# SimonRennotte/Data-Efficient-Reinforcement-Learning-with-Probabilistic-Model-Predictive-Control

Hardware: AMD Instinct MI355X
Metric: MPC trajectory rollouts/sec (higher is better)
Workload: dtype f64

## Files before the change

### data-efficient-reinforcement-learning-with-probabilistic-model-predictive-control_amd/csrc/rollout_kernel.h

```cpp
#pragma once
#include "device_common.h"

#if defined(GPMPC_PROF_ON)
#define GPMPC_TRACE(id) do { if (threadIdx.x == 0 && blockIdx.x == 0) { long long now_ = __builtin_readcyclecounter(); \
    prof_acc[id] += now_ - prof_last; prof_last = now_; } \
    if (CL && threadIdx.x == 0 && (blockIdx.x & 7) == 0) { long long w_ = wall_clock64(); prof_wall[id] += w_ - prof_wlast; prof_wlast = w_; } } while (0)
#else
#define GPMPC_TRACE(id) do {} while (0)
#endif

namespace gpmpc_hip {

typedef const __attribute__((address_space(3))) double* lds_cptr;
__device__ inline double lds_b64(const double* p) {
    lds_cptr q = (lds_cptr)p;
    asm volatile("" : "+v"(q));
    return *q;
}

typedef double lds_d2 __attribute__((ext_vector_type(2)));
template <int NL, int NV>
__device__ inline void lds_load_pairs(const double* rec, double (&v)[NV]) {
    static_assert(NV >= ((NL + 1) & ~1), "destination too short");
    const lds_d2* r2 = reinterpret_cast<const lds_d2*>(rec);
#pragma unroll
    for (int k = 0; k < (NL + 1) / 2; ++k) { const lds_d2 t = r2[k]; v[2 * k] = t.x; v[2 * k + 1] = t.y; }
}

template <int DP>
struct RowRecPacked {
    static constexpr int RS = DP + 2, EA = 0, RA = 1, G = 2;
    template <int NL>
    static __device__ inline void load(const double* rec, double (&v)[RS]) {
#pragma unroll
        for (int k = 0; k < NL; ++k) v[k] = rec[k];
    }
};
template <int DP>
struct RowRecAligned {
    static constexpr int RS = (DP + 3) & ~1, EA = DP, RA = DP + 1, G = 0;
    template <int NL>
    static __device__ inline void load(const double* rec, double (&v)[RS]) { lds_load_pairs<NL>(rec, v); }
};

constexpr int kMaxTaylor = 14;
constexpr int kMaxMono = 256;

constexpr int kLaneMapSlots = 32;
constexpr int kLaneMapSlotsCluster = 192;
__host__ __device__ inline int tri_ints(int N) { return (N + 7) / 8 + 2; }

struct Layout {
    int mu, Sig, m, M, cc, s1, Vs, Sp, misc, rdet, aug, part, mom, ints, lmap, cl;
    int c_ils2, c_logvar, c_var, c_xr, c_act, c_exptab, c_monow, c_monoe, c_X;
    int lds_total;
    int nu, lb, rows, kb;
    int pp_total;
};

__host__ __device__ inline int rnd2(int x) { return (x + 1) & ~1; }

constexpr int kClusterScratch = 16 * 64 / 8;

__host__ __device__ inline Layout make_layout(int N, int D, int A, int E, int G, int DP, int wpp, int CM, int CH, int HA,
                                              bool x_in_lds, bool cluster = false, int lds_pairs = 0) {
    const int GL = (cluster && lds_pairs > 0) ? lds_pairs : G;
    Layout L;
    const int P = D * (D + 1) / 2;
    int o = 0;
    L.mu = o;   o += rnd2(D);
    L.Sig = o;  o += 2 * rnd2(D * D);
    L.m = o;    o += rnd2(E);
    L.M = o;    o += rnd2(D);
    L.cc = o;   o += rnd2(D);
    L.s1 = o;   o += rnd2(D * (D + 1));
    L.Vs = o;   o += rnd2(D * D);
    L.Sp = o;   o += rnd2(P);
    L.misc = o; o += 8;
    L.rdet = o; o += rnd2(G);
    L.aug = o;  o += (D + G) * 2 * D * D;
    L.part = o; o += rnd2(G * wpp);
    L.mom = o;  o += G * 2 * rnd2(CM);
    L.ints = o; o += rnd2((2 * P + 3 * G + 8 + 16 + tri_ints(N) + 1) / 2) + rnd2((D + G * wpp + 3) / 4);
    const int lms = cluster ? kLaneMapSlotsCluster : kLaneMapSlots;
    L.lmap = o; o += rnd2(((wpp < lms ? wpp : lms) * 65 + 1) / 2);
    L.cl = o;       o += cluster ? rnd2(G) + rnd2((G + 1) / 2) + 2 + kClusterScratch + rnd2((G * wpp + 2 * G + 16 + 7) / 8) +
                                   rnd2((G * wpp + 16 + 4 + 3) / 4) + rnd2((G + 1) / 2) + rnd2(G) : 0;
    L.c_ils2 = o;   o += rnd2(D * E);
    L.c_logvar = o; o += rnd2(D);
    L.c_var = o;    o += rnd2(D);
    L.c_xr = o;     o += rnd2(2 * E);
    L.c_act = o;    o += rnd2(HA);
    L.c_exptab = o; o += 64;
    L.c_monow = o;  o += rnd2(CM);
    L.c_monoe = o;  o += rnd2((CM + 1) / 2);
    L.c_X = o;      o += x_in_lds ? rnd2(E * N) : 0;
    int q = o;
    L.nu = q;   q += rnd2(D * N);
    L.lb = q;   q += rnd2(D * N);
    L.rows = q; q += GL * (N + CH) * ((DP + 3) & ~1);
    L.kb = q;   q += rnd2(GL * N);
    L.lds_total = q;
    L.pp_total = q - o;
    return L;
}

__device__ inline double gauss_solve(double* aug, int D, int nrhs, int ld) {
    double det = 1.0;
    const int nc = D + nrhs;
    for (int k = 0; k < D; ++k) {
        int piv = k;
        double best = fabs(aug[k * ld + k]);
        for (int r = k + 1; r < D; ++r) {
            double v = fabs(aug[r * ld + k]);
            if (v > best) { best = v; piv = r; }
        }
        if (piv != k) {
            for (int c = k; c < nc; ++c) {
                double t = aug[k * ld + c];
                aug[k * ld + c] = aug[piv * ld + c];
                aug[piv * ld + c] = t;
            }
            det = -det;
        }
        const double pv = aug[k * ld + k];
        det *= pv;
        const double ip = 1.0 / pv;
        for (int r = k + 1; r < D; ++r) {
            const double f = aug[r * ld + k] * ip;
            for (int c = k + 1; c < nc; ++c) aug[r * ld + c] -= f * aug[k * ld + c];
        }
    }
    for (int k = D - 1; k >= 0; --k) {
        const double ip = 1.0 / aug[k * ld + k];
        for (int c = D; c < nc; ++c) {
            double s = aug[k * ld + c];
            for (int r = k + 1; r < D; ++r) s -= aug[k * ld + r] * aug[r * ld + c];
            aug[k * ld + c] = s * ip;
        }
    }
    return det;
}

template <int DP>
__device__ inline double gauss_solve_reg(double (&a)[DP][2 * DP]) {
    double det = 1.0;
#pragma unroll
    for (int k = 0; k < DP; ++k) {
        int piv = k;
        double best = fabs(a[k][k]);
#pragma unroll
        for (int r = k + 1; r < DP; ++r) {
            const double v = fabs(a[r][k]);
            const bool better = v > best;
            best = better ? v : best;
            piv = better ? r : piv;
        }
#pragma unroll
        for (int r = k + 1; r < DP; ++r) {
            const bool sw = (piv == r);
#pragma unroll
            for (int c = 0; c < 2 * DP; ++c) {
                const double x = a[k][c], y = a[r][c];
                a[k][c] = sw ? y : x;
                a[r][c] = sw ? x : y;
            }
// ... 418 lines not shown
            const double(&grp)[16] = *reinterpret_cast<const double(*)[16]>(&acc[g16]);
            const double tot = wave_reduce16(grp);
            if ((lane & 3) == 0 && g16 + mq < NBm) mom[canon.v[g16 + mq]] = tot;
        }
        if constexpr (NP % 16 != 0) {
            constexpr int g8 = NP - 8;
            const double(&grp)[8] = *reinterpret_cast<const double(*)[8]>(&acc[g8]);
            const double tot = wave_reduce8(grp);
            if ((lane & 3) == 0 && lane < 32 && g8 + mq < NBm) mom[canon.v[g8 + mq]] = tot;
        }
    }
}

template <int KS>
__device__ __attribute__((noinline)) void sep3_item(int band, int lane, int N, int side, const double* rec0, int RS,
                                                     const double* kb, const double* nu, const double* il, double* mom) {
    switch (band) {
        case 0: sep3_band<KS, 0>(lane, N, side, rec0, RS, kb, nu, il, mom); break;
        case 1: sep3_band<KS, 1>(lane, N, side, rec0, RS, kb, nu, il, mom); break;
        case 2: sep3_band<KS, 2>(lane, N, side, rec0, RS, kb, nu, il, mom); break;
        case 3: sep3_band<KS, 3>(lane, N, side, rec0, RS, kb, nu, il, mom); break;
        case 4: sep3_band<KS, 4>(lane, N, side, rec0, RS, kb, nu, il, mom); break;
        case 5: sep3_band<KS, 5>(lane, N, side, rec0, RS, kb, nu, il, mom); break;
        default: sep3_band<KS, 6>(lane, N, side, rec0, RS, kb, nu, il, mom); break;
    }
}

template <int DP, bool CL>
constexpr int rollout_min_waves() { return (DP == 2 || (DP == 3 && !CL)) ? 4 : (DP == 6 ? 3 : 1); }

template <int DP, int NT, int DX, bool C2, bool TILED = false, bool CL = false>
__global__ __launch_bounds__(NT, (rollout_min_waves<DP, CL>())) void rollout_kernel(const RolloutArgs p) {
    static_assert(!TILED || (DP <= 4 && NT >= 256), "the batch-major path is built for D <= 4");
    static_assert(!CL || (!TILED && DP <= 4 && NT >= 256), "the cooperative form is built for D <= 4");
    extern __shared__ __attribute__((aligned(16))) double smem[];
    if constexpr (TILED) {
        if (p.slow[blockIdx.x] != p.t_begin + 1) return;
    }
    constexpr int NW = NT / kWave;
    using REC = RowRecAligned<DP>;
    constexpr int RS = REC::RS;
    const int tid = threadIdx.x;
    const int CS = CL ? p.cluster : 1;
    const bool spread = CL && (p.cl_dbg & 8);
    const int member = CL ? (spread ? (int)blockIdx.x % CS : (int)(blockIdx.x >> 3) % CS) : 0;
    const int c = CL ? (spread ? (int)blockIdx.x / CS : (int)(blockIdx.x & 7) + 8 * ((int)(blockIdx.x >> 3) / CS)) : (int)blockIdx.x;
    if constexpr (CL) { if (c >= p.B) return; }
    constexpr bool kMerged = !CL && DX > 0 && DP <= 4;
    constexpr bool kTailInTrip = DX == 0 || DP > 4;
    const int D = (DX > 0) ? DX : p.D;
    const int N = p.N, A = p.A, E = p.E, H = p.H, G = p.G, CM = p.CM;
    const int P = TILED ? D * (D - 1) / 2 : D * (D + 1) / 2;
    const int DA = D + A;
    const int LD = 2 * D;
    const int NC = C2 ? (N + 1) / 2 : N;
    const int wpp = (p.RC * NC + 63) / 64;
    const int SD2 = rnd2(D * D);

    const Layout L = make_layout(N, D, A, E, G, DP, wpp, CM, p.CH, H * A, p.x_in_lds != 0, CL, CL ? p.cl_slots : 0);
    const int NR = N + p.CH;
    double* s_mu = smem + L.mu;
    double* s_Sig2 = smem + L.Sig;
    double* s_m = smem + L.m;
    double* s_M = smem + L.M;
    double* s_cc = smem + L.cc;
    double* s_s1 = smem + L.s1;
    double* s_Vs = smem + L.Vs;
    double* s_Sp = smem + L.Sp;
    double* s_rdet = smem + L.rdet;
    [[maybe_unused]] double* s_rdiag = smem + L.misc;
    double* s_aug = smem + L.aug;
    double* s_part = smem + L.part;
    double* s_mom = smem + L.mom;
    int* s_pa = reinterpret_cast<int*>(smem + L.ints);
    int* s_pb = s_pa + P;
    int* s_K = s_pb + P;
    int* s_counter = s_K + G;
    int* s_noff = s_counter + 1;
    int* s_off = s_noff + 1;
    int* s_mcum = s_off + G;
    int* s_tri = s_mcum + 16;
    int* s_nslot = s_tri + tri_ints(N);
    int* s_nitems = s_nslot + G;
    unsigned short* s_items = reinterpret_cast<unsigned short*>(
        smem + L.ints + rnd2((2 * P + 3 * G + 8 + 16 + tri_ints(N) + 1) / 2));

    [[maybe_unused]] double* s_sepv = smem + L.cl;
    [[maybe_unused]] int* s_ord = reinterpret_cast<int*>(smem + L.cl + rnd2(G));
    [[maybe_unused]] int* s_fail = reinterpret_cast<int*>(smem + L.cl + rnd2(G) + rnd2((G + 1) / 2));
    [[maybe_unused]] unsigned char* s_needw = reinterpret_cast<unsigned char*>(smem + L.cl + rnd2(G) + rnd2((G + 1) / 2) + 2);
    [[maybe_unused]] unsigned char* s_own = s_needw + kClusterScratch * 8;
    [[maybe_unused]] unsigned char* s_sepown = s_own + G * wpp;
    [[maybe_unused]] unsigned char* s_elneed = s_sepown + G;
    [[maybe_unused]] unsigned char* s_meanown = s_elneed + G;
    [[maybe_unused]] unsigned short* s_mine = reinterpret_cast<unsigned short*>(
        smem + L.cl + rnd2(G) + rnd2((G + 1) / 2) + 2 + kClusterScratch + rnd2((G * wpp + 2 * G + 16 + 7) / 8));
    [[maybe_unused]] int* s_slot = reinterpret_cast<int*>(smem + L.cl + rnd2(G) + rnd2((G + 1) / 2) + 2 + kClusterScratch +
                                                          rnd2((G * wpp + 2 * G + 16 + 7) / 8) + rnd2((G * wpp + 16 + 4 + 3) / 4));
    [[maybe_unused]] unsigned long long* s_mymask = reinterpret_cast<unsigned long long*>(
        smem + L.cl + rnd2(G) + rnd2((G + 1) / 2) + 2 + kClusterScratch + rnd2((G * wpp + 2 * G + 16 + 7) / 8) +
        rnd2((G * wpp + 16 + 4 + 3) / 4) + rnd2((G + 1) / 2));
    const int GL = CL ? p.cl_slots : G;

    [[maybe_unused]] unsigned long long* xbuf_uc = CL ? p.xch_uc + (size_t)c * 4 * p.xch_n : nullptr;
    [[maybe_unused]] unsigned long long* xbuf = CL ? p.xch + (size_t)c * 4 * p.xch_n : nullptr;
    [[maybe_unused]] const int x_sep = G * wpp, x_mean = G * wpp + G;
    [[maybe_unused]] const int x_xcc = x_mean + D * (D + 1);
    [[maybe_unused]] int* s_lmap = reinterpret_cast<int*>(smem + L.lmap);
    constexpr int LMS = CL ? kLaneMapSlotsCluster : kLaneMapSlots;
    [[maybe_unused]] int* s_lrows = s_lmap + (wpp < LMS ? wpp : LMS) * 64;
    double* ppbase = smem;
    double* a_nu = ppbase + L.nu;
    double* a_lb = ppbase + L.lb;
    double* a_rows = ppbase + L.rows;
    double* a_kb = ppbase + L.kb;

    double* c_ils2 = smem + L.c_ils2;
    double* c_logvar = smem + L.c_logvar;
    double* c_var = smem + L.c_var;
    double* c_xr = smem + L.c_xr;
    double* c_act = smem + L.c_act;
    double* c_exptab = smem + L.c_exptab;
    const double* Xs = p.x_in_lds ? (smem + L.c_X) : p.Xt;
    double* c_monow = smem + L.c_monow;
    int* c_monoe = reinterpret_cast<int*>(smem + L.c_monoe);
    const double* act = p.actions + (size_t)c * H * A;

#if defined(GPMPC_PROF_ON)
    long long prof_left = 0;
    long long prof_acc[10] = {0, 0, 0, 0, 0, 0, 0, 0, 0, 0};
    long long prof_last = __builtin_readcyclecounter();
    long long prof_wall[10] = {0, 0, 0, 0, 0, 0, 0, 0, 0, 0};
    long long prof_wlast = wall_clock64();
    long long prof_b3 = 0, prof_chain = 0;
    int prof_chain_n = 0;
#endif
    if constexpr (TILED) {
        for (int i = tid; i < D; i += NT) { s_mu[i] = p.mu_out[((size_t)c * (H + 1) + p.t_begin) * D + i]; c_logvar[i] = p.logvar[i]; c_var[i] = p.var[i]; }
        for (int i = tid; i < D * D; i += NT) s_Sig2[i] = p.Sig_out[((size_t)c * (H + 1) + p.t_begin) * D * D + i];
    }
    {
        const bool inl = p.act_inline_n > 0;
        const int CMc = CM > 0 ? CM : 0;
        const double* mw = CMc > 0 ? p.mono_w : p.ils2;
        const int* me = CMc > 0 ? p.mono_exp : reinterpret_cast<const int*>(p.ils2);
        const int im = tid < CMc ? tid : 0;
        const int nX = p.x_in_lds ? E * N : 0;
        __builtin_amdgcn_sched_barrier(0);
        const double v_lv = p.logvar[tid < D ? tid : 0], v_var = p.var[tid < D ? tid : 0];
        const double v_ils = p.ils2[tid < D * E ? tid : 0], v_xr = p.xrange[tid < 2 * E ? tid : 0];
        const double v_act = act[tid < H * A ? tid : 0];
        const double v_exp = kExp2Tab[tid & 63];
        const double v_mw = mw[im];
        const int e0 = me[im * 4], e1 = me[im * 4 + 1], e2 = me[im * 4 + 2], e3 = me[im * 4 + 3];
        const double v_x0 = p.Xt[tid < nX ? tid : 0], v_x1 = p.Xt[tid + NT < nX ? tid + NT : 0];
        [[maybe_unused]] const double v_mu0 = p.mu0[tid < D ? tid : 0], v_S0 = p.S0[tid < D * D ? tid : 0];
        __builtin_amdgcn_sched_barrier(0);
        if constexpr (!TILED) {
            if (tid < D) s_mu[tid] = v_mu0;
            if (tid < D * D) s_Sig2[tid] = v_S0;
        }
        if (tid < D) { c_logvar[tid] = v_lv; c_var[tid] = v_var; }
        if (tid < D * E) c_ils2[tid] = v_ils;
        if (tid < 2 * E) c_xr[tid] = v_xr;
        if (tid < 64) c_exptab[tid] = v_exp;
        if (tid < CMc) { c_monow[tid] = v_mw; c_monoe[tid] = e0 | (e1 << 8) | (e2 << 16) | (e3 << 24); }
        if (tid < nX) smem[L.c_X + tid] = v_x0;
        if (tid + NT < nX) smem[L.c_X + tid + NT] = v_x1;
        if (inl) {
            for (int i = tid; i < H * A; i += NT) {
                const double v = p.act_inline[i < kInlineActs ? i : 0];
                c_act[i] = v;
                if (!CL || member == 0) p.act_store[i] = v;
            }
        } else {
            if (tid < H * A) c_act[tid] = v_act;
            for (int i = tid + NT; i < H * A; i += NT) c_act[i] = act[i];
        }
        for (int i = tid + NT; i < D; i += NT) { c_logvar[i] = p.logvar[i]; c_var[i] = p.var[i]; }
        for (int i = tid + NT; i < D * E; i += NT) c_ils2[i] = p.ils2[i];
        for (int i = tid + NT; i < 2 * E; i += NT) c_xr[i] = p.xrange[i];
        for (int i = tid + 2 * NT; i < nX; i += NT) smem[L.c_X + i] = p.Xt[i];
        for (int i = tid + NT; i < CMc; i += NT) {
            c_monow[i] = p.mono_w[i];
            c_monoe[i] = p.mono_exp[i * 4] | (p.mono_exp[i * 4 + 1] << 8) | (p.mono_exp[i * 4 + 2] << 16) | (p.mono_exp[i * 4 + 3] << 24);
        }
    }
    for (int i = tid; i < GL * p.CH * RS; i += NT) {
        const int gq = i / (p.CH * RS), k = i - gq * (p.CH * RS);
        a_rows[((size_t)gq * NR + N) * RS + k] = 0.0;
    }
    if (tid >= 64 && tid < 80) s_mcum[tid - 64] = p.mono_cum[tid - 64];
    if (tid == 0) {
        int q = 0;
        [[maybe_unused]] int nd_ = 0, no_ = 0;
        for (int a = 0; a < D; ++a)
            for (int b = TILED ? a + 1 : a; b < D; ++b) {
                s_pa[q] = a; s_pb[q] = b;
                if constexpr (CL) s_ord[q] = (a == b) ? nd_++ : no_++;
                ++q;
            }
        if constexpr (CL) *s_fail = 0;
        int run = 0;
        for (int r = 0; r <= p.RC; ++r) {
            s_tri[r] = run;
            const int first = C2 ? (r * p.CH) / 2 : r * p.CH;
            run += (first < NC) ? NC - first : 0;
        }
    }
    __syncthreads();
    bool use_lmap = false;
    if constexpr (!TILED) {
        const int wtri = (s_tri[p.RC] + 63) >> 6;
        use_lmap = wtri <= LMS && wtri <= wpp;
        if (use_lmap) {
            for (int slot = tid >> 6; slot < wtri; slot += NW) {
                const int flat = slot * 64 + (tid & 63);
                const bool valid = flat < s_tri[p.RC];
// ... 431 lines not shown
                }
#if defined(GPMPC_PROF_ON)
                if (threadIdx.x == 0 && blockIdx.x == 0) { long long now_ = __builtin_readcyclecounter(); prof_acc[7] += now_ - prof_last; }
                if (blockIdx.x == 0 && (threadIdx.x == 0 || threadIdx.x == kPairBase) && prof_b3 != 0) {
                    prof_chain += __builtin_readcyclecounter() - prof_b3;
                    ++prof_chain_n;
                }
#endif
            }
            if (step_done) { traj_mu += D; traj_Sig += D * D; }
            if (!more) break;
            if constexpr (TILED) {
                if (first && tid >= 128 && tid < 128 + D) {
                    const int a = tid - 128;
                    double m[DP][2 * DP];
#pragma unroll
                    for (int i = 0; i < DP; ++i)
#pragma unroll
                        for (int j = 0; j < DP; ++j) {
                            const bool in = (i < D && j < D);
                            const double sg = in ? s_Sig[i * D + j] : 0.0;
                            const double dab = in ? c_ils2[a * E + j] + c_ils2[a * E + j] : 0.0;
                            m[i][j] = sg * dab + (i == j ? 1.0 : 0.0);
                            m[i][DP + j] = sg;
                        }
                    s_rdiag[a] = 1.0 / sqrt(small_solve<DP>(m));
                } else if (first && wave == 3) {
                    for (int a = 0; a < D; ++a) {
                        const double* tp = p.tile_part + ((size_t)c * D + a) * p.ntiles;
                        double v = 0.0;
                        for (int k = lane; k < p.ntiles; k += 64) v += tp[k];
                        v = wave_sum(v);
                        if (lane == 0) s_rdiag[4 + a] = v;
                    }
                }
            }
            if (tid == NT - 1) {
                *s_counter = 0;
                int no = 0;
                for (int gq = 0; gq < Gc; ++gq)
                    if (s_pa[q0 + gq] != s_pb[q0 + gq]) s_off[no++] = gq;
                *s_noff = no;
            }
            __syncthreads();
            GPMPC_TRACE(2);

            const int n_off = *s_noff;
            [[maybe_unused]] bool cl_list_pending = false;
            [[maybe_unused]] int cl_ns = 0, cl_cls = 3, cl_code0 = 0;
            if (wave == NW - 1) {
                const int wtri = (s_tri[p.RC] + 63) >> 6;
                const int R = Gc + nmean;
                int ns = 0, cls = 3, code0 = 0;
                [[maybe_unused]] unsigned long long mymask = 0;
                if (lane < Gc) {
                    const int Kr = s_K[lane];
                    const bool sep = (Kr & 64) != 0;
                    if (sep) {
                        const int Ks = Kr & 63;
                        const int two = (DX == 3) ? 2 * sep3_bands(Ks <= 3 ? 3 : Ks) : 2 * ((s_mcum[Ks] + 7) >> 3);
                        ns = two < wpp ? two : wpp;
                    } else {
                        ns = (s_pa[q0 + lane] == s_pb[q0 + lane]) ? wtri : wpp;
                    }
                    cls = sep ? 1 : 0;
                    code0 = lane * wpp;
                    s_nslot[lane] = ns;
                    if constexpr (CL) {
                        if (sep) mymask = (s_sepown[lane] == member) ? (ns >= 64 ? ~0ull : (1ull << ns) - 1ull) : 0ull;
                        else mymask = s_mymask[lane];
                    }
                } else if (lane < R) {
                    ns = 1; cls = 2; code0 = 0xffff - (lane - Gc);
                    if constexpr (CL) mymask = (s_meanown[lane - Gc] == member) ? 1ull : 0ull;
                }
                auto build_list = [&] {
                    int start = 0, total_items = 0;
                    for (int m = 0; m < R; ++m) {
                        const int nsm = __builtin_amdgcn_readlane(ns, m);
                        const int clm = __builtin_amdgcn_readlane(cls, m);
                        start += (clm < cls || (clm == cls && m < lane)) ? nsm : 0;
                        total_items += nsm;
                    }
                    for (int k = 0; k < ns; ++k) s_items[start + k] = (unsigned short)(cls == 2 ? code0 : code0 + k);
                    if (lane == 0) *s_nitems = total_items;
                    return total_items;
                };
                if constexpr (!CL) {
                    (void)build_list();
                } else if (wpp > 64) {
                    const int total_items = build_list();
                    wave_lds_sync();
                    int cnt = 0;
                    for (int base = 0; base < total_items; base += 64) {
                        const int k = base + lane;
                        const int code = s_items[k < total_items ? k : 0];
                        const bool mine = k < total_items && item_owner(code) == member;
                        const unsigned long long mask = __ballot(mine);
                        if (mine) s_mine[1 + cnt + __popcll(mask & ((1ull << lane) - 1ull))] = (unsigned short)code;
                        cnt += __popcll(mask);
                    }
                    if (lane == 0) s_mine[0] = (unsigned short)cnt;
                } else {
                    const int mycnt = __popcll(mymask);
                    int pre = 0, tot = 0, total_items = 0;
                    for (int m = 0; m < R; ++m) {
                        const int cm = __builtin_amdgcn_readlane(mycnt, m);
                        const int clm = __builtin_amdgcn_readlane(cls, m);
                        pre += (clm < cls || (clm == cls && m < lane)) ? cm : 0;
                        tot += cm;
                        total_items += __builtin_amdgcn_readlane(ns, m);
                    }
                    unsigned long long mk = mymask;
                    for (int i = 0; mk != 0; ++i) {
                        const int k = __builtin_ctzll(mk);
                        mk &= mk - 1ull;
                        s_mine[1 + pre + i] = (unsigned short)(cls == 2 ? code0 : code0 + k);
                    }
                    if (lane == 0) { s_mine[0] = (unsigned short)tot; *s_nitems = total_items; }
                    cl_list_pending = true;
                    cl_ns = ns; cl_cls = cls; cl_code0 = code0;
                }
            }
            const int p2_threads = (NW >= 8) ? NT - 64 : NT;
            int p2_items = (nmean + Gc + n_off) * N;
            [[maybe_unused]] bool cl_nu_first = false;
            if (CL && (NW < 8 || wave != NW - 1)) {
                const int nall = nmean + Gc + n_off;
                bool need = false;
                int code = lane;
                if (lane < nmean) need = s_meanown[lane] == member;
                else if (lane < nmean + Gc) need = pair_needed(lane - nmean);
                else if (lane < nall) need = pair_needed(s_off[lane - nmean - Gc]);
                const unsigned long long mask0 = __ballot(need);
                if (lane == nall) { need = s_meanown[0] != member && mask0 == 0; code = 255; }
                const unsigned long long mask = __ballot(need);
                if (need) s_needw[wave * 64 + __popcll(mask & ((1ull << lane) - 1ull))] = (unsigned char)code;
                p2_items = __popcll(mask) * N;
                cl_nu_first = s_meanown[0] != member && mask0 != 0;
                wave_lds_sync();
            }
            for (int it = tid; it < p2_items && tid < p2_threads; it += p2_threads) {
                int prob = p.magic_pt ? (int)__umulhi((unsigned)it, p.magic_pt) : it;
                const int pt = it - prob * N;
                double nu[DP];
#pragma unroll
                for (int d = 0; d < DP; ++d) nu[d] = (d < D) ? (Xs[d * N + pt] - s_m[d]) : 0.0;
                if constexpr (CL) {
                    if (cl_nu_first && prob == 0) {
#pragma unroll
                        for (int d = 0; d < DP; ++d)
                            if (d < D) a_nu[d * N + pt] = nu[d];
                    }
                    prob = s_needw[wave * 64 + prob];
                    if (prob == 255) {
#pragma unroll
                        for (int d = 0; d < DP; ++d)
                            if (d < D) a_nu[d * N + pt] = nu[d];
                        continue;
                    }
                }
                if (prob < nmean) {
                    const int a = prob;
                    const double* Ai = s_aug + a * (D * LD) + D;
                    double q = 0.0;
#pragma unroll
                    for (int i = 0; i < DP; ++i) {
// ... 16 lines not shown
                            if (d < D) a_nu[d * N + pt] = nu[d];
                    }
                } else {
                    const bool rowside = prob < nmean + Gc;
                    const int gq = rowside ? prob - nmean : s_off[prob - nmean - Gc];
                    const int a = s_pa[q0 + gq], b = s_pb[q0 + gq];
                    const int c = rowside ? a : b;
                    const int Kw = s_K[gq];
                    const int K = Kw & 63;
                    const int sl = CL ? (Kw >> 8) - 1 : gq;
                    const double* Z = s_aug + (D + gq) * (D * LD) + D;
                    double u[DP], g[DP];
                    double ks = 0.0;
#pragma unroll
                    for (int d = 0; d < DP; ++d) {
                        u[d] = nu[d] * ((d < D) ? c_ils2[c * E + d] : 0.0);
                        ks = fma(nu[d], u[d], ks);
                        g[d] = 0.0;
                    }
                    for (int e = D; e < E; ++e) {
                        const double v = Xs[e * N + pt] - s_m[e];
                        ks = fma(v * v, c_ils2[c * E + e], ks);
                    }
                    double qq = 0.0;
#pragma unroll
                    for (int i = 0; i < DP; ++i) {
                        if (i < D) {
                            double zu = 0.0;
#pragma unroll
                            for (int j = 0; j < DP; ++j)
                                if (j < D) {
                                    const double z = Z[i * LD + j];
                                    zu = fma(z, u[j], zu);
                                    g[j] = fma(z, u[i], g[j]);
                                }
                            qq = fma(u[i], zu, qq);
                        }
                    }
                    const double kk = c_logvar[c] - 0.5 * ks + 0.5 * qq;
                    const double bc = p.beta[c * N + pt];
                    if (rowside) {
                        double* rec = a_rows + ((size_t)sl * NR + pt) * RS;
#pragma unroll
                        for (int d = 0; d < DP; ++d) rec[REC::G + d] = g[d];
                        if (K > 0) {
                            const double ea = fast_exp(kk, c_exptab);
                            rec[REC::EA] = ea;
                            rec[REC::RA] = ea * bc;
                            if (a == b) a_kb[sl * N + pt] = ea;
                        } else {
                            rec[REC::EA] = kk;
                            rec[REC::RA] = bc;
                            if (a == b) a_kb[sl * N + pt] = kk;
                        }
                        if constexpr (REC::RS > DP + 2) rec[DP + 2] = 0.0;
                    } else {
                        a_kb[sl * N + pt] = (K > 0) ? fast_exp(kk, c_exptab) * bc : kk;
                    }
                }
            }
            __syncthreads();
            GPMPC_TRACE(3);

            const int total = *s_nitems;
            if constexpr (CL) {
                if (cl_list_pending) {
                    const int R = Gc + nmean;
                    int start = 0;
                    for (int m = 0; m < R; ++m) {
                        const int nsm = __builtin_amdgcn_readlane(cl_ns, m);
                        const int clm = __builtin_amdgcn_readlane(cl_cls, m);
                        start += (clm < cl_cls || (clm == cl_cls && m < lane)) ? nsm : 0;
                    }
                    for (int m = 0; m < R; ++m) {
                        const int nsm = __builtin_amdgcn_readlane(cl_ns, m), sm = __builtin_amdgcn_readlane(start, m);
                        const int clm = __builtin_amdgcn_readlane(cl_cls, m), c0 = __builtin_amdgcn_readlane(cl_code0, m);
                        if (lane < nsm) s_items[sm + lane] = (unsigned short)(clm == 2 ? c0 : c0 + lane);
                    }
                }
            }
#if defined(GPMPC_PROF_ON)
            const long long prof_p3 = __builtin_readcyclecounter();
#endif
            auto pull_item = [&]() -> int {
                int pulled = 0;
                if (lane == 0) {
                    pulled = __hip_atomic_fetch_add(s_counter, 1, __ATOMIC_RELAXED, __HIP_MEMORY_SCOPE_WORKGROUP);
                    pulled = (pulled < total) ? (int)s_items[pulled] : -1;
                }
                return __builtin_amdgcn_readfirstlane(pulled);
            };
            [[maybe_unused]] int cl_next = wave;
            [[maybe_unused]] const int cl_count = CL ? (int)s_mine[0] : 0;
            auto next_item = [&]() -> int {
                if constexpr (!CL) return pull_item();
                else {
                    if (cl_next >= cl_count) return -1;
                    const int code = __builtin_amdgcn_readfirstlane((int)s_mine[1 + cl_next]);
                    cl_next += NW;
                    return code;
                }
            };
            for (int wq = next_item(); wq >= 0; wq = next_item()) {
                if (wq >= 0xffff - 15) {
                    const int a = 0xffff - wq;
                    for (int dd = 0; dd <= D; ++dd) {
                        double v = 0.0;
                        if (dd == 0) { for (int pt = lane; pt < N; pt += 64) v += a_lb[a * N + pt]; }
                        else { for (int pt = lane; pt < N; pt += 64) v = fma(a_lb[a * N + pt], a_nu[(dd - 1) * N + pt], v); }
                        v = wave_sum(v);
                        if (lane == 0) {
                            s_s1[a * (D + 1) + dd] = v;
                            if constexpr (CL) publish(x_mean + a * (D + 1) + dd, v);
                        }
                    }
                    continue;
                }
                const int wi = wq;
                const int gq = p.magic_wpp ? (int)__umulhi((unsigned)wi, p.magic_wpp) : wi;
                const int slot = wi - gq * wpp;
                const int a = __builtin_amdgcn_readfirstlane(s_pa[q0 + gq]);
                const int b = __builtin_amdgcn_readfirstlane(s_pb[q0 + gq]);
                const int Kraw = __builtin_amdgcn_readfirstlane(s_K[gq]);
                const int K = Kraw & 63;
                const bool diag = (a == b);
                if (Kraw & 64) {
                    [[maybe_unused]] const int sl3 = CL ? (Kraw >> 8) - 1 : gq;
                    if constexpr (DX == 3) {
                        const int KS = K <= 3 ? 3 : K;
                        const int nbands = sep3_bands(KS);
                        for (int itm = slot; itm < 2 * nbands; itm += wpp) {
                            const int side = itm >= nbands, band = itm - side * nbands;
                            const double* rec0 = a_rows + (size_t)sl3 * NR * RS;
                            const double* kbp = a_kb + sl3 * N;
                            const double* il = c_ils2 + b * E;
                            double* mom = s_mom + (gq * 2 + side) * rnd2(CM);
                            if (K <= 3) sep3_item<3>(band, lane, N, side, rec0, RS, kbp, a_nu, il, mom);
                            else if (K == 4) sep3_item<4>(band, lane, N, side, rec0, RS, kbp, a_nu, il, mom);
                            else if (K == 5) sep3_item<5>(band, lane, N, side, rec0, RS, kbp, a_nu, il, mom);
                            else sep3_item<6>(band, lane, N, side, rec0, RS, kbp, a_nu, il, mom);
                        }
                        continue;
                    }
                    const int C = s_mcum[K];
                    const int NBk = (C + 7) >> 3;
                    for (int blk = slot; blk < 2 * NBk; blk += wpp) {
                        const int side = blk >= NBk;
                        const int al0 = (blk - side * NBk) * 8;
                        int packed[8];
#pragma unroll
                        for (int m = 0; m < 8; ++m) packed[m] = __builtin_amdgcn_readfirstlane((al0 + m < C) ? c_monoe[al0 + m] : 0);
                        double acc[8];
#pragma unroll
                        for (int m = 0; m < 8; ++m) acc[m] = 0.0;
                        for (int pt = lane; pt < N; pt += 64) {
                            double x[DP];
                            double wt;
                            if (side == 0) {
                                double r[RS];
                                REC::template load<RS>(a_rows + ((size_t)sl3 * NR + pt) * RS, r);
                                wt = r[REC::RA];
#pragma unroll
                                for (int d = 0; d < DP; ++d) x[d] = r[REC::G + d];
                            } else {
                                wt = a_kb[sl3 * N + pt];
#pragma unroll
                                for (int d = 0; d < DP; ++d) x[d] = (d < D) ? a_nu[d * N + pt] * c_ils2[b * E + d] : 0.0;
                            }
#pragma unroll
                            for (int m = 0; m < 8; ++m) {
                                double t = wt;
#pragma unroll
                                for (int d = 0; d < (DP < 4 ? DP : 4); ++d) {
                                    const int ne = (packed[m] >> (8 * d)) & 255;
                                    for (int e = 0; e < ne; ++e) t *= x[d];
                                }
                                acc[m] += t;
                            }
                        }
                        const double tot = wave_reduce8(acc);
                        const int mm = lane >> 2;
                        if ((lane & 3) == 0 && lane < 32 && al0 + mm < C) s_mom[(gq * 2 + side) * rnd2(CM) + al0 + mm] = tot;
                    }
                    continue;
                }
                const int flat = slot * 64 + lane;
                bool valid;
                int r, jc;
                int nrows_tab = -1;
                if (diag && use_lmap) {
                    const int packed = s_lmap[flat];
                    valid = packed >= 0;
                    r = valid ? (packed & 255) : 0;
                    jc = valid ? (packed >> 8) : 0;
                    nrows_tab = __builtin_amdgcn_readfirstlane(s_lrows[slot]);
                } else if (diag) {
                    valid = flat < s_tri[p.RC];
                    int lo = 0, hi = p.RC;
                    while (hi - lo > 1) {
                        const int mid = (lo + hi) >> 1;
                        if (s_tri[mid] <= flat) lo = mid; else hi = mid;
                    }
                    r = valid ? lo : 0;
                    const int first = C2 ? (r * p.CH) / 2 : r * p.CH;
                    jc = valid ? first + (flat - s_tri[r]) : 0;
                } else {
                    valid = flat < p.RC * NC;
                    r = valid ? (p.magic_N ? (int)__umulhi((unsigned)flat, p.magic_N) : flat) : 0;
                    jc = valid ? flat - r * NC : 0;
                }
                const int j = C2 ? 2 * jc : jc;
                const bool valid1 = C2 && (j + 1 < N);
                const int jl = valid1 ? j + 1 : j;
                const int i0 = r * p.CH;
                int i1 = i0 + p.CH;
                if (i1 > N) i1 = N;
                if (diag && i1 > jl + 1) i1 = jl + 1;
                int nrows = nrows_tab;
                if (nrows_tab < 0) {
                    const int len = (valid && i1 > i0) ? (i1 - i0) : 0;
                    nrows = (wave_max_i32(len) + 3) & ~3;
                }
                double acc = 0.0;
                if (nrows > 0) {
                    double w[DP];
#pragma unroll
                    for (int d = 0; d < DP; ++d) w[d] = (d < D) ? a_nu[d * N + j] * c_ils2[b * E + d] : 0.0;
                    const int sle = CL ? (Kraw >> 8) - 1 : gq;
                    const double kbj = a_kb[sle * N + j];
                    const double* rec = a_rows + ((size_t)sle * NR + i0) * RS;
                    [[maybe_unused]] const double* Tp = p.Tm + ((size_t)a * (N + kTPad) + i0) * N + j;
                    if constexpr (C2) {
                        const TRows trows = make_t_rows(p.Tm, D, N, a, i0, j);
                        double w1[DP];
                        const double m1 = valid1 ? 1.0 : 0.0;
#pragma unroll
                        for (int d = 0; d < DP; ++d) w1[d] = (d < D) ? a_nu[d * N + jl] * (c_ils2[b * E + d] * m1) : 0.0;
                        const double kb1 = a_kb[sle * N + jl] * m1;
                        double acc0, acc1;
                        if (K == 0) {
                            item_exp2<DP>(rec, nrows, w, w1, kbj, kb1, diag, trows, c_exptab, acc0, acc1);
                            acc = acc0 * (diag ? 2.0 : p.beta[b * N + j]) + (valid1 ? acc1 * (diag ? 2.0 : p.beta[b * N + j + 1]) : 0.0);
                        } else {
                            constexpr int TU = DP >= 4 ? 4 : 2;
                            if (K <= 2) item_taylor2<DP, 2, TU>(rec, nrows, w, w1, diag, trows, acc0, acc1);
                            else if (K == 3) item_taylor2<DP, 3, TU>(rec, nrows, w, w1, diag, trows, acc0, acc1);
                            else if (K == 4) item_taylor2<DP, 4, TU>(rec, nrows, w, w1, diag, trows, acc0, acc1);
                            else if (K == 5) item_taylor2<DP, 5, TU>(rec, nrows, w, w1, diag, trows, acc0, acc1);
                            else if (K == 6) item_taylor2<DP, 6, TU>(rec, nrows, w, w1, diag, trows, acc0, acc1);
                            else if (K == 7) item_taylor2<DP, 7, TU>(rec, nrows, w, w1, diag, trows, acc0, acc1);
                            else if (K == 8) item_taylor2<DP, 8, TU>(rec, nrows, w, w1, diag, trows, acc0, acc1);
                            else if (K <= 10) item_taylor2<DP, 10, TU>(rec, nrows, w, w1, diag, trows, acc0, acc1);
                            else if (K <= 12) item_taylor2<DP, 12, TU>(rec, nrows, w, w1, diag, trows, acc0, acc1);
                            else item_taylor2<DP, 14, TU>(rec, nrows, w, w1, diag, trows, acc0, acc1);
                            acc = fma(acc0, kbj, acc1 * kb1) * (diag ? 2.0 : 1.0);
                        }
                    } else if (K == 0) {
                        acc = item_exp<DP, REC>(rec, nrows, w, kbj, diag, Tp, N, c_exptab);
                        acc *= diag ? 2.0 : p.beta[b * N + j];
                    } else {
                        if (K <= 2) acc = item_taylor<DP, 2, REC>(rec, nrows, w, diag, Tp, N);
                        else if (K == 3) acc = item_taylor<DP, 3, REC>(rec, nrows, w, diag, Tp, N);
                        else if (K == 4) acc = item_taylor<DP, 4, REC>(rec, nrows, w, diag, Tp, N);
                        else if (K == 5) acc = item_taylor<DP, 5, REC>(rec, nrows, w, diag, Tp, N);
                        else if (K == 6) acc = item_taylor<DP, 6, REC>(rec, nrows, w, diag, Tp, N);
                        else if (K == 7) acc = item_taylor<DP, 7, REC>(rec, nrows, w, diag, Tp, N);
                        else if (K == 8) acc = item_taylor<DP, 8, REC>(rec, nrows, w, diag, Tp, N);
                        else if (K <= 10) acc = item_taylor<DP, 10, REC>(rec, nrows, w, diag, Tp, N);
                        else if (K <= 12) acc = item_taylor<DP, 12, REC>(rec, nrows, w, diag, Tp, N);
                        else acc = item_taylor<DP, 14, REC>(rec, nrows, w, diag, Tp, N);
                        acc *= diag ? 2.0 * kbj : kbj;
                    }
                    acc = valid ? acc : 0.0;
                }
                acc = wave_sum(acc);
                if (lane == 0) {
                    s_part[wi] = acc;
                    if constexpr (CL) publish(wi, acc);
                }
            }
#if defined(GPMPC_PROF_ON) && defined(GPMPC_PROF_BARRIER)
            if constexpr (CL) __syncthreads();
#endif
            GPMPC_TRACE(8);
            if constexpr (CL) {
                const bool own_sep = __ballot(lane < Gc && (s_K[lane < Gc ? lane : 0] & 64) && s_sepown[lane < Gc ? lane : 0] == member) != 0;
                __syncthreads();
                if (own_sep) {
                    for (int gq = wave; gq < Gc; gq += NW) {
                        const int Kraw = s_K[gq];
                        if (!(Kraw & 64) || s_sepown[gq] != member) continue;
                        const int C = s_mcum[Kraw & 63];
                        const double* Gm = s_mom + (gq * 2) * rnd2(CM);
                        const double* Wm = Gm + rnd2(CM);
                        double v = 0.0;
                        for (int al = lane; al < C; al += 64) v = fma(Gm[al] * Wm[al], c_monow[al], v);
                        v = wave_sum(v);
                        if (lane == 0) publish(x_sep + gq, v);
                    }
                }
                const int npair = total - nmean;
                for (int k = tid; k < npair + nmean * (D + 1); k += NT) {
                    int vi = -1;
                    double* dst = nullptr;
                    if (k < npair) {
                        const int code = s_items[k];
                        const int gq = p.magic_wpp ? (int)__umulhi((unsigned)code, p.magic_wpp) : code;
                        if (!(s_K[gq] & 64)) { vi = code; dst = s_part + code; }
                        else if (code == gq * wpp) { vi = x_sep + gq; dst = s_sepv + gq; }
                    } else {
                        vi = x_mean + (k - npair); dst = s_s1 + (k - npair);
                    }
                    if (vi >= 0) *dst = acquire(vi);
                }
            }
#if defined(GPMPC_PROF_ON)
            if (blockIdx.x == 0 && (threadIdx.x & 63) == 0) prof_left += __builtin_readcyclecounter() - prof_p3;
#endif
            __syncthreads();
            GPMPC_TRACE(4);
#if defined(GPMPC_PROF_ON)
            if (blockIdx.x == 0 && (threadIdx.x & 63) == 0 && threadIdx.x <= 64) prof_b3 = __builtin_readcyclecounter();
#endif
            if constexpr (CL) {
                if (*s_fail) {
                    if (member == 0) {
                        for (int i = tid; i < (H - t) * D; i += NT) p.mu_out[((size_t)c * (H + 1) + (t + 1)) * D + i] = __builtin_nan("");
                        for (int i = tid; i < (H - t) * D * D; i += NT) p.Sig_out[((size_t)c * (H + 1) + (t + 1)) * D * D + i] = __builtin_nan("");
                    }
                    return;
                }
            }
            if constexpr (kTailInTrip) {
                for (int gq = wave; gq < Gc; gq += NW) {
                    const int Kraw = s_K[gq];
                    double v = 0.0;
                    if ((Kraw & 64) && CL) {
                        v = s_sepv[gq];
                    } else {
                        if (Kraw & 64) {
                            const int C = s_mcum[Kraw & 63];
                            const double* Gm = s_mom + (gq * 2) * rnd2(CM);
                            const double* Wm = Gm + rnd2(CM);
                            for (int al = lane; al < C; al += 64) v = fma(Gm[al] * Wm[al], c_monow[al], v);
                        } else {
                            const int ns = s_nslot[gq];
                            for (int k = lane; k < ns; k += 64) v += s_part[gq * wpp + k];
                        }
                        v = wave_sum(v);
                    }
                    if constexpr (TILED) {
                        const int a = s_pa[q0 + gq], b = s_pb[q0 + gq];
                        if (lane == 0) s_Sp[a * D - (a * (a - 1)) / 2 + (b - a)] = v * s_rdet[gq];
                    } else {
                        if (lane == 0) s_Sp[q0 + gq] = v * s_rdet[gq];
                    }
                }
                if constexpr (TILED) {
                    if (first && tid < D) s_Sp[tid * D - (tid * (tid - 1)) / 2] = 2.0 * s_rdiag[4 + tid] * s_rdiag[tid];
                }
                if (first) {
                    if (tid < D) s_M[tid] = s_cc[tid] * s_s1[tid * (D + 1)];
                    for (int idx = tid; idx < D * D; idx += NT) {
                        const int k = idx / D, a = idx - k * D;
                        const double* Ai = s_aug + a * (D * LD) + D;
                        double s = 0.0;
                        for (int j = 0; j < D; ++j) s = fma(Ai[k * LD + j], s_s1[a * (D + 1) + 1 + j], s);
                        s_Vs[idx] = s_cc[a] * s;
                    }
                }
                __syncthreads();
                GPMPC_TRACE(5);
                if (q0 + G >= P) {
                    double* s_SigNext = s_Sig2 + (cur ^ 1) * SD2;
                    for (int idx = tid; idx < D * D; idx += NT) {
                        const int i = idx / D, j = idx - i * D;
                        const int a = i < j ? i : j, b = i < j ? j : i;
                        const int q = a * D - (a * (a - 1)) / 2 + (b - a);
                        const double S = s_Sp[q] - s_M[i] * s_M[j] + (i == j ? c_var[i] : 0.0);
                        double cij = 0.0, cji = 0.0;
                        for (int k = 0; k < D; ++k) {
                            cij = fma(s_Sig[i * D + k], s_Vs[k * D + j], cij);
                            cji = fma(s_Sig[j * D + k], s_Vs[k * D + i], cji);
                        }
                        const double v = S + s_Sig[idx] + (cij + cji);
                        s_SigNext[idx] = v;
                        if (member == 0) p.Sig_out[((size_t)c * (H + 1) + (t + 1)) * D * D + idx] = v;
                    }
                    for (int i = tid; i < D; i += NT) {
                        const double v = s_mu[i] + s_M[i];
                        s_mu[i] = v;
                        if (member == 0) p.mu_out[((size_t)c * (H + 1) + (t + 1)) * D + i] = v;
                    }
                    cur ^= 1;
                    __syncthreads();
                    GPMPC_TRACE(6);
                }
            }
        }
        if constexpr (!kTailInTrip) have_prev = true;
        pq0 = q0;
        q0 += G;
        if (q0 >= P) { q0 = 0; ++t; }
    }
#if defined(GPMPC_PROF_ON)
    if (threadIdx.x == 0 && blockIdx.x == 0) printf("PROF wave0 small algebra cycles %lld\n", prof_acc[7]);
    if (blockIdx.x == 0 && (threadIdx.x & 63) == 0 && prof_chain_n > 0)
        printf("PROF chain wave %d: end of P3 -> arrival at the P1 barrier %lld cycles over %d intervals\n", (int)(threadIdx.x >> 6), prof_chain, prof_chain_n);
    if (blockIdx.x == 0 && (threadIdx.x & 63) == 0) printf("PROF P3 wave %d left the queue after %lld\n", (int)(threadIdx.x >> 6), prof_left);
    if (CL && threadIdx.x == 0 && (blockIdx.x & 7) == 0)
        printf("PROF member %2d xcc %d same_xcd %d\n", member, (int)__builtin_amdgcn_s_getreg(20 | (0 << 6) | ((4 - 1) << 11)), (int)same_xcd);
    if (CL && threadIdx.x == 0 && (blockIdx.x & 7) == 0)
        printf("PROF member %2d wall (10 ns ticks): P1 %lld | P2 %lld | items(wave 0) %lld | gather+wait %lld | P4 %lld | P5 %lld\n", member,
               prof_wall[2], prof_wall[3], prof_wall[8], prof_wall[4], prof_wall[5], prof_wall[6]);
    if (threadIdx.x == 0 && blockIdx.x == 0)
        printf("PROF cycles: init %lld | P1 %lld | P2 %lld | P3 %lld (wave 0's items %lld) | P4 %lld | P5 %lld\n", prof_acc[1], prof_acc[2],
               prof_acc[3], prof_acc[4] + prof_acc[8], prof_acc[8], prof_acc[5], prof_acc[6]);
#endif
}

__device__ __forceinline__ void traj_cost_generic(int c, int lane, const double* __restrict__ mu, const double* __restrict__ Sig,
                                                          const double* __restrict__ actions, const double* __restrict__ cost,
                                                          int D, int A, int H, double kappa, int clip, int use_constraints,
                                                          double* __restrict__ cm_out, double* __restrict__ cv_out,
                                                          double* __restrict__ J_out) {
    const int DA = D + A;
    const double* target = cost;
    const double* W = cost + DA;
    const double* WT = W + DA * DA;
    const double* smin = WT + D * D;
    const double* smax = smin + D;
    double jsum = 0.0;
    for (int t = lane; t <= H; t += 64) {
        const bool terminal = (t == H);
        const int n = terminal ? D : DA;
        const double* Wm = terminal ? WT : W;
        const double* m = mu + ((size_t)c * (H + 1) + t) * D;
        const double* S = Sig + ((size_t)c * (H + 1) + t) * D * D;
        const double* a = actions + ((size_t)c * H + (terminal ? 0 : t)) * A;
        auto err = [&](int i) { return (i < D ? m[i] : a[i - D]) - target[i]; };
        double cm = 0.0, cv = 0.0;
        for (int i = 0; i < D; ++i)
            for (int j = 0; j < D; ++j) cm = fma(S[i * D + j], Wm[j * n + i], cm);
        for (int i = 0; i < n; ++i) {
            const double ei = err(i);
            for (int j = 0; j < n; ++j) cm = fma(ei * Wm[i * n + j], err(j), cm);
        }
        for (int i = 0; i < D; ++i)
            for (int j = 0; j < D; ++j) {
                double tij = 0.0, tji = 0.0;
                for (int k = 0; k < D; ++k) {
                    tij = fma(Wm[i * n + k], S[k * D + j], tij);
                    tji = fma(Wm[j * n + k], S[k * D + i], tji);
                }
                cv = fma(2.0 * tij, tji, cv);
                double v1 = 0.0, v2 = 0.0;
                for (int k = 0; k < n; ++k) {
                    v1 = fma(err(k), Wm[k * n + i], v1);
                    v2 = fma(Wm[j * n + k], err(k), v2);
                }
                cv = fma(4.0 * v1 * S[i * D + j], v2, cv);
            }
        if (use_constraints && !terminal) {
            for (int d = 0; d < D; ++d) {
                const double sg = S[d * D + d];
                cm += 0.5 * (1.0 + erf((smin[d] - m[d]) / (sg * 1.4142135623730951)))
                    + (1.0 - 0.5 * (1.0 + erf((smax[d] - m[d]) / (sg * 1.4142135623730951))));
            }
        }
        double ucb = -cm + kappa * sqrt(cv);
        if (clip) ucb = fmin(ucb, 0.0);
        jsum -= ucb;
        if (cm_out) cm_out[(size_t)c * (H + 1) + t] = cm;
        if (cv_out) cv_out[(size_t)c * (H + 1) + t] = cv;
    }
    jsum = wave_xor_sum(jsum);
    if (lane == 0 && J_out) J_out[c] = jsum / (double)(H + 1);
}

template <int D, int N>
__device__ __forceinline__ void stage_cost_terms(const double* S, const double* e, const double* Wm, double& cm_out, double& cv_out) {
    double cm = 0.0, cv = 0.0;
#pragma unroll
    for (int i = 0; i < D; ++i)
#pragma unroll
        for (int j = 0; j < D; ++j) cm = fma(S[i * D + j], Wm[j * N + i], cm);
#pragma unroll
    for (int i = 0; i < N; ++i) {
        const double ei = e[i];
#pragma unroll
        for (int j = 0; j < N; ++j) cm = fma(ei * Wm[i * N + j], e[j], cm);
    }
// ... 99 lines not shown
```

Baseline: 736,700.

## Pack per-item descriptors in the work queue and prefetch the next claim

For the non-cluster DP==3 path, the item list now holds packed 64-bit descriptors (code, table row count, K, slot, pair index, a, b) instead of 16-bit codes. Each wave then decodes its item from one LDS read instead of doing a magic-number divide and several dependent LDS loads. The atomic claim of the next queue index is also issued early, right after an item's main loop, so its latency overlaps the wave reduction. The descriptor array costs more LDS, and optional profiling instrumentation is added for per-item head, loop and tail timing.

```diff
diff --git a/data-efficient-reinforcement-learning-with-probabilistic-model-predictive-control_amd/csrc/rollout_kernel.h b/data-efficient-reinforcement-learning-with-probabilistic-model-predictive-control_amd/csrc/rollout_kernel.h
--- a/data-efficient-reinforcement-learning-with-probabilistic-model-predictive-control_amd/csrc/rollout_kernel.h
+++ b/data-efficient-reinforcement-learning-with-probabilistic-model-predictive-control_amd/csrc/rollout_kernel.h
@@ -61,6 +61,13 @@
 __host__ __device__ inline int rnd2(int x) { return (x + 1) & ~1; }
 
 constexpr int kClusterScratch = 16 * 64 / 8;
+
+__host__ __device__ inline unsigned item_desc_lo(int code, int nrows_tab, int Kraw) {
+    return (unsigned)code | ((unsigned)(nrows_tab + 1) << 16) | ((unsigned)(Kraw & 127) << 24);
+}
+__host__ __device__ inline unsigned item_desc_hi(int slot, int gq, int a, int b) {
+    return (unsigned)slot | ((unsigned)gq << 16) | ((unsigned)a << 22) | ((unsigned)b << 26);
+}
 
 __host__ __device__ inline Layout make_layout(int N, int D, int A, int E, int G, int DP, int wpp, int CM, int CH, int HA,
                                               bool x_in_lds, bool cluster = false, int lds_pairs = 0) {
@@ -81,7 +88,7 @@
     L.aug = o;  o += (D + G) * 2 * D * D;
     L.part = o; o += rnd2(G * wpp);
     L.mom = o;  o += G * 2 * rnd2(CM);
-    L.ints = o; o += rnd2((2 * P + 3 * G + 8 + 16 + tri_ints(N) + 1) / 2) + rnd2((D + G * wpp + 3) / 4);
+    L.ints = o; o += rnd2((2 * P + 3 * G + 8 + 16 + tri_ints(N) + 1) / 2) + ((cluster || DP != 3) ? rnd2((D + G * wpp + 3) / 4) : rnd2(D + G * wpp));
     const int lms = cluster ? kLaneMapSlotsCluster : kLaneMapSlots;
     L.lmap = o; o += rnd2(((wpp < lms ? wpp : lms) * 65 + 1) / 2);
     L.cl = o;       o += cluster ? rnd2(G) + rnd2((G + 1) / 2) + 2 + kClusterScratch + rnd2((G * wpp + 2 * G + 16 + 7) / 8) +
@@ -666,8 +673,10 @@
     int* s_tri = s_mcum + 16;
     int* s_nslot = s_tri + tri_ints(N);
     int* s_nitems = s_nslot + G;
-    unsigned short* s_items = reinterpret_cast<unsigned short*>(
+    [[maybe_unused]] unsigned short* s_items = reinterpret_cast<unsigned short*>(
         smem + L.ints + rnd2((2 * P + 3 * G + 8 + 16 + tri_ints(N) + 1) / 2));
+    constexpr bool kDesc = !CL && DP == 3;
+    [[maybe_unused]] uint2* s_desc = reinterpret_cast<uint2*>(smem + L.ints + rnd2((2 * P + 3 * G + 8 + 16 + tri_ints(N) + 1) / 2));
 
     [[maybe_unused]] double* s_sepv = smem + L.cl;
     [[maybe_unused]] int* s_ord = reinterpret_cast<int*>(smem + L.cl + rnd2(G));
@@ -718,6 +727,9 @@
     long long prof_wlast = wall_clock64();
     long long prof_b3 = 0, prof_chain = 0;
     int prof_chain_n = 0;
+    long long prof_ih[3] = {0, 0, 0}, prof_il[3] = {0, 0, 0}, prof_it[3] = {0, 0, 0};
+    int prof_in[3] = {0, 0, 0}, prof_icls = -1;
+    long long prof_ipull = 0, prof_ifirst = 0, prof_ilast = 0;
 #endif
     if constexpr (TILED) {
         for (int i = tid; i < D; i += NT) { s_mu[i] = p.mu_out[((size_t)c * (H + 1) + p.t_begin) * D + i]; c_logvar[i] = p.logvar[i]; c_var[i] = p.var[i]; }
@@ -1315,7 +1327,18 @@
                         start += (clm < cls || (clm == cls && m < lane)) ? nsm : 0;
                         total_items += nsm;
                     }
-                    for (int k = 0; k < ns; ++k) s_items[start + k] = (unsigned short)(cls == 2 ? code0 : code0 + k);
+                    if constexpr (!kDesc) {
+                        for (int k = 0; k < ns; ++k) s_items[start + k] = (unsigned short)(cls == 2 ? code0 : code0 + k);
+                    } else {
+                        int pa = 0, pb = 0, Kr = 0;
+                        if (cls < 2) { pa = s_pa[q0 + lane]; pb = s_pb[q0 + lane]; Kr = s_K[lane]; }
+                        const bool tab = cls == 0 && pa == pb && use_lmap;
+                        for (int k = 0; k < ns; ++k) {
+                            const int code = cls == 2 ? code0 : code0 + k;
+                            const int nrt = tab ? s_lrows[k] : -1;
+                            s_desc[start + k] = make_uint2(item_desc_lo(code, nrt, Kr), item_desc_hi(k, lane, pa, pb));
+                        }
+                    }
                     if (lane == 0) *s_nitems = total_items;
                     return total_items;
                 };
@@ -1498,28 +1521,67 @@
 #if defined(GPMPC_PROF_ON)
             const long long prof_p3 = __builtin_readcyclecounter();
 #endif
-            auto pull_item = [&]() -> int {
-                int pulled = 0;
-                if (lane == 0) {
-                    pulled = __hip_atomic_fetch_add(s_counter, 1, __ATOMIC_RELAXED, __HIP_MEMORY_SCOPE_WORKGROUP);
-                    pulled = (pulled < total) ? (int)s_items[pulled] : -1;
-                }
-                return __builtin_amdgcn_readfirstlane(pulled);
+            [[maybe_unused]] int q_nidx = 0;
+            [[maybe_unused]] bool q_claimed = false;
+            [[maybe_unused]] int wq_hi = 0;
+            auto q_claim = [&]() -> int {
+                typedef __attribute__((address_space(3))) int* lds_iptr;
+                lds_iptr cq = (lds_iptr)s_counter;
+                asm volatile("" : "+v"(cq));
+                int i = 0;
+                if (lane == 0) i = __hip_atomic_fetch_add(cq, 1, __ATOMIC_RELAXED, __HIP_MEMORY_SCOPE_WORKGROUP);
+                return i;
             };
+            [[maybe_unused]] auto q_claim_late = [&] { q_nidx = q_claim(); q_claimed = true; };
             [[maybe_unused]] int cl_next = wave;
             [[maybe_unused]] const int cl_count = CL ? (int)s_mine[0] : 0;
             auto next_item = [&]() -> int {
-                if constexpr (!CL) return pull_item();
-                else {
+                if constexpr (!CL && !kDesc) {
+                    int pulled = 0;
+                    if (lane == 0) {
+                        pulled = __hip_atomic_fetch_add(s_counter, 1, __ATOMIC_RELAXED, __HIP_MEMORY_SCOPE_WORKGROUP);
+                        pulled = (pulled < total) ? (int)s_items[pulled] : -1;
+                    }
+                    return __builtin_amdgcn_readfirstlane(pulled);
+                } else if constexpr (kDesc) {
+                    if (!q_claimed) q_nidx = q_claim();
+                    q_claimed = false;
+                    uint2 d = make_uint2(~0u, 0u);
+                    if (lane == 0 && q_nidx < total) d = s_desc[q_nidx];
+                    wq_hi = __builtin_amdgcn_readfirstlane((int)d.y);
+                    return __builtin_amdgcn_readfirstlane((int)d.x);
+                } else {
                     if (cl_next >= cl_count) return -1;
                     const int code = __builtin_amdgcn_readfirstlane((int)s_mine[1 + cl_next]);
                     cl_next += NW;
                     return code;
                 }
             };
-            for (int wq = next_item(); wq >= 0; wq = next_item()) {
-                if (wq >= 0xffff - 15) {
-                    const int a = 0xffff - wq;
+#if defined(GPMPC_PROF_ON)
+            prof_icls = -1;
+            auto next_item_prof = [&]() -> int {
+                const long long now_ = __builtin_readcyclecounter();
+                if (prof_icls >= 0) {
+                    prof_ih[prof_icls] += prof_ifirst - prof_ipull; prof_il[prof_icls] += prof_ilast - prof_ifirst;
+                    prof_it[prof_icls] += now_ - prof_ilast; ++prof_in[prof_icls];
+                }
+                prof_icls = -1;
+                prof_ipull = now_;
+                return next_item();
+            };
+#define GPMPC_NEXT_ITEM next_item_prof
+#define GPMPC_ITEM_FIRST(cls) do { prof_icls = (cls); prof_ifirst = __builtin_readcyclecounter(); prof_ilast = prof_ifirst; } while (0)
+#define GPMPC_ITEM_LAST() do { prof_ilast = __builtin_readcyclecounter(); } while (0)
+#else
+#define GPMPC_NEXT_ITEM next_item
+#define GPMPC_ITEM_FIRST(cls) do {} while (0)
+#define GPMPC_ITEM_LAST() do {} while (0)
+#endif
+            for (int wq = GPMPC_NEXT_ITEM(); wq >= 0; wq = GPMPC_NEXT_ITEM()) {
+                const int wi = kDesc ? (wq & 0xffff) : wq;
+                if (wi >= 0xffff - 15) {
+                    const int a = 0xffff - wi;
+                    GPMPC_ITEM_FIRST(2);
                     for (int dd = 0; dd <= D; ++dd) {
                         double v = 0.0;
                         if (dd == 0) { for (int pt = lane; pt < N; pt += 64) v += a_lb[a * N + pt]; }
@@ -1530,14 +1592,21 @@
                             if constexpr (CL) publish(x_mean + a * (D + 1) + dd, v);
                         }
                     }
+                    GPMPC_ITEM_LAST();
                     continue;
                 }
-                const int wi = wq;
-                const int gq = p.magic_wpp ? (int)__umulhi((unsigned)wi, p.magic_wpp) : wi;
-                const int slot = wi - gq * wpp;
-                const int a = __builtin_amdgcn_readfirstlane(s_pa[q0 + gq]);
-                const int b = __builtin_amdgcn_readfirstlane(s_pb[q0 + gq]);
-                const int Kraw = __builtin_amdgcn_readfirstlane(s_K[gq]);
+                int gq, slot, a, b, Kraw;
+                [[maybe_unused]] int desc_nrows = -1;
+                if constexpr (!kDesc) {
+                    gq = p.magic_wpp ? (int)__umulhi((unsigned)wi, p.magic_wpp) : wi;
+                    slot = wi - gq * wpp;
+                    a = __builtin_amdgcn_readfirstlane(s_pa[q0 + gq]);
+                    b = __builtin_amdgcn_readfirstlane(s_pb[q0 + gq]);
+                    Kraw = __builtin_amdgcn_readfirstlane(s_K[gq]);
+                } else {
+                    slot = wq_hi & 0xffff; gq = (wq_hi >> 16) & 63; a = (wq_hi >> 22) & 15; b = (wq_hi >> 26) & 15;
+                    Kraw = (wq >> 24) & 127; desc_nrows = ((wq >> 16) & 255) - 1;
+                }
                 const int K = Kraw & 63;
                 const bool diag = (a == b);
                 if (Kraw & 64) {
@@ -1545,6 +1614,7 @@
                     if constexpr (DX == 3) {
                         const int KS = K <= 3 ? 3 : K;
                         const int nbands = sep3_bands(KS);
+                        GPMPC_ITEM_FIRST(1);
                         for (int itm = slot; itm < 2 * nbands; itm += wpp) {
                             const int side = itm >= nbands, band = itm - side * nbands;
                             const double* rec0 = a_rows + (size_t)sl3 * NR * RS;
@@ -1556,10 +1626,12 @@
                             else if (K == 5) sep3_item<5>(band, lane, N, side, rec0, RS, kbp, a_nu, il, mom);
                             else sep3_item<6>(band, lane, N, side, rec0, RS, kbp, a_nu, il, mom);
                         }
+                        GPMPC_ITEM_LAST();
                         continue;
                     }
                     const int C = s_mcum[K];
                     const int NBk = (C + 7) >> 3;
+                    GPMPC_ITEM_FIRST(1);
                     for (int blk = slot; blk < 2 * NBk; blk += wpp) {
                         const int side = blk >= NBk;
                         const int al0 = (blk - side * NBk) * 8;
@@ -1598,6 +1670,7 @@
                         const int mm = lane >> 2;
                         if ((lane & 3) == 0 && lane < 32 && al0 + mm < C) s_mom[(gq * 2 + side) * rnd2(CM) + al0 + mm] = tot;
                     }
+                    GPMPC_ITEM_LAST();
                     continue;
                 }
                 const int flat = slot * 64 + lane;
@@ -1609,7 +1682,8 @@
                     valid = packed >= 0;
                     r = valid ? (packed & 255) : 0;
                     jc = valid ? (packed >> 8) : 0;
-                    nrows_tab = __builtin_amdgcn_readfirstlane(s_lrows[slot]);
+                    if constexpr (!kDesc) nrows_tab = __builtin_amdgcn_readfirstlane(s_lrows[slot]);
+                    else nrows_tab = desc_nrows;
                 } else if (diag) {
                     valid = flat < s_tri[p.RC];
                     int lo = 0, hi = p.RC;
@@ -1654,6 +1728,7 @@
                         for (int d = 0; d < DP; ++d) w1[d] = (d < D) ? a_nu[d * N + jl] * (c_ils2[b * E + d] * m1) : 0.0;
                         const double kb1 = a_kb[sle * N + jl] * m1;
                         double acc0, acc1;
+                        GPMPC_ITEM_FIRST(0);
                         if (K == 0) {
                             item_exp2<DP>(rec, nrows, w, w1, kbj, kb1, diag, trows, c_exptab, acc0, acc1);
                             acc = acc0 * (diag ? 2.0 : p.beta[b * N + j]) + (valid1 ? acc1 * (diag ? 2.0 : p.beta[b * N + j + 1]) : 0.0);
@@ -1672,9 +1747,11 @@
                             acc = fma(acc0, kbj, acc1 * kb1) * (diag ? 2.0 : 1.0);
                         }
                     } else if (K == 0) {
+                        GPMPC_ITEM_FIRST(0);
                         acc = item_exp<DP, REC>(rec, nrows, w, kbj, diag, Tp, N, c_exptab);
                         acc *= diag ? 2.0 : p.beta[b * N + j];
                     } else {
+                        GPMPC_ITEM_FIRST(0);
                         if (K <= 2) acc = item_taylor<DP, 2, REC>(rec, nrows, w, diag, Tp, N);
                         else if (K == 3) acc = item_taylor<DP, 3, REC>(rec, nrows, w, diag, Tp, N);
                         else if (K == 4) acc = item_taylor<DP, 4, REC>(rec, nrows, w, diag, Tp, N);
@@ -1687,7 +1764,11 @@
                         else acc = item_taylor<DP, 14, REC>(rec, nrows, w, diag, Tp, N);
                         acc *= diag ? 2.0 * kbj : kbj;
                     }
+                    GPMPC_ITEM_LAST();
+                    if constexpr (kDesc) q_claim_late();
                     acc = valid ? acc : 0.0;
+                } else {
+                    GPMPC_ITEM_FIRST(0);
                 }
                 acc = wave_sum(acc);
                 if (lane == 0) {
@@ -1695,6 +1776,9 @@
                     if constexpr (CL) publish(wi, acc);
                 }
             }
+#undef GPMPC_NEXT_ITEM
+#undef GPMPC_ITEM_FIRST
+#undef GPMPC_ITEM_LAST
 #if defined(GPMPC_PROF_ON) && defined(GPMPC_PROF_BARRIER)
             if constexpr (CL) __syncthreads();
 #endif
@@ -1824,6 +1908,10 @@
     if (blockIdx.x == 0 && (threadIdx.x & 63) == 0 && prof_chain_n > 0)
         printf("PROF chain wave %d: end of P3 -> arrival at the P1 barrier %lld cycles over %d intervals\n", (int)(threadIdx.x >> 6), prof_chain, prof_chain_n);
     if (blockIdx.x == 0 && (threadIdx.x & 63) == 0) printf("PROF P3 wave %d left the queue after %lld\n", (int)(threadIdx.x >> 6), prof_left);
+    if (blockIdx.x == 0 && (threadIdx.x & 63) == 0)
+        printf("PROF items wave %2d: element-wise n %d head %lld loop %lld tail %lld | separable n %d head %lld loop %lld tail %lld | mean n %d head %lld loop %lld tail %lld\n",
+               (int)(threadIdx.x >> 6), prof_in[0], prof_ih[0], prof_il[0], prof_it[0], prof_in[1], prof_ih[1], prof_il[1], prof_it[1],
+               prof_in[2], prof_ih[2], prof_il[2], prof_it[2]);
     if (CL && threadIdx.x == 0 && (blockIdx.x & 7) == 0)
         printf("PROF member %2d xcc %d same_xcd %d\n", member, (int)__builtin_amdgcn_s_getreg(20 | (0 << 6) | ((4 - 1) << 11)), (int)same_xcd);
     if (CL && threadIdx.x == 0 && (blockIdx.x & 7) == 0)
```

New measurement: 757,200 (median of 6 runs). 2.8% higher.
